# rsjahnige/CRYSTALS-Kyber

Measured on NVIDIA B200. Metric: ML-KEM-768 Encaps+Decaps ops/s, higher is better.
Workload: dtype u16/u64 integer

## Files before the change

### crystals-kyber_b200/csrc/mlkem_b200.cu

```cuda
#include "mlkem_kernels.cuh"

#include "../../include/mlkem_b200.h"

#include <algorithm>
#include <atomic>
#include <cstdio>
#include <cstdlib>
#include <cstring>
#include <mutex>
#include <vector>

namespace {

using namespace mlkem;

thread_local char tl_error[512] = "";
std::atomic<unsigned long long> g_launches{0};
int env_int(const char *name, int dflt) {
    const char *v = getenv(name);
    return v && *v ? atoi(v) : dflt;
}
constexpr int kSlots = 6;
constexpr int kDevSlots = 4;
constexpr int kHostSlots = 3;
// ... 65 lines not shown
    for (int i = 0; i < 7; i++) o |= ((r >> i) & 1u) << (6 - i);
    return o;
}
unsigned pow17(unsigned e) {
    unsigned z = 1;
    while (e--) z = (z * 17u) % kQ;
    return z;
}
uint2 shoup_pair(unsigned w) { return make_uint2(w, (w << 16) / kQ); }
uint2 shoup_pair32(unsigned w) { return make_uint2(w, (unsigned)(((unsigned long long)w << 32) / kQ)); }

void build_tables(TwiddleTables &t, uint2 rc[24]) {
    for (unsigned i = 0; i < 128; i++) {
        t.zeta[i] = shoup_pair(pow17(bitrev7(i)));
        t.gamma[i] = shoup_pair(pow17(2 * bitrev7(i) + 1));
        t.gamma32[i] = shoup_pair32(t.gamma[i].x);
        t.zeta32[i] = shoup_pair32(t.zeta[i].x);
    }
    t.zeta_inv_last[0] = shoup_pair((t.zeta[1].x * 3303u) % kQ);
    t.zeta_inv_last[1] = shoup_pair(3303u);
    t.zeta_inv_last32[0] = shoup_pair32(t.zeta_inv_last[0].x);
    t.zeta_inv_last32[1] = shoup_pair32(3303u);
    uint8_t lfsr = 1;
    for (int round = 0; round < 24; round++) {
        unsigned long long c = 0;
        for (int j = 0; j <= 6; j++) {
            if (lfsr & 1) c |= 1ULL << ((1u << j) - 1);
            uint8_t hi = lfsr & 0x80;
            lfsr = (uint8_t)(lfsr << 1);
            if (hi) lfsr ^= 0x71;
        }
        rc[round] = make_uint2((unsigned)c, (unsigned)(c >> 32));
    }
}

struct DeviceCtx {
    bool ready = false;
    cudaStream_t stream[kSlots] = {};
    void *ws[kSlots] = {};
    size_t ws_bytes[kSlots] = {};
    void *io[kSlots] = {};
    size_t io_bytes[kSlots] = {};
    cudaEvent_t ev_fork = nullptr, ev_join[kSlots] = {}, ev_slot[kSlots] = {};
    void *misc = nullptr;
    size_t misc_bytes = 0;
    int host_group = 0;
    std::mutex call_mutex;
    std::mutex misc_mutex;
};
DeviceCtx g_ctx[kMaxDevices];
std::mutex g_mutex;

struct DeviceGuard {
    int prev = -1;
    bool changed = false;
    int enter(int d) {
        if (cudaGetDevice(&prev) != cudaSuccess) prev = -1;
        if (prev == d) return 0;
        CU(cudaSetDevice(d));
        changed = true;
        return 0;
    }
    ~DeviceGuard() {
        if (changed && prev >= 0) cudaSetDevice(prev);
    }
};

// ... 19 lines not shown
    return 0;
}
template <class P>
int allow_smem_matvec() {
    const size_t b = matvec_smem_bytes<P>();
    if (int rc = allow_smem(k_sample_matvec<P, kModeKeyGen>, b)) return rc;
    if (int rc = allow_smem(k_sample_matvec<P, kModeEncrypt>, b)) return rc;
    if (int rc = allow_smem(k_sample_matvec<P, kModeEncryptCompare>, b)) return rc;
    if (int rc = allow_smem(k_sample_matvec_list<P, kModeKeyGen>, b)) return rc;
    if (int rc = allow_smem(k_sample_matvec_list<P, kModeEncrypt>, b)) return rc;
    if (int rc = allow_smem(k_sample_matvec_list<P, kModeEncryptCompare>, b)) return rc;
    return 0;
}

int acquire(const mlkem_b200_opts *o, int *dev, DeviceCtx **ctx, DeviceGuard &guard) {
    int d = o ? o->device : -1;
    if (d < 0) CU(cudaGetDevice(&d));
    if (d >= kMaxDevices) {
        snprintf(tl_error, sizeof tl_error, "device ordinal %d out of range", d);
        return MLKEM_B200_ERR_ARG;
    }
    if (int rc = guard.enter(d)) return rc;
    std::lock_guard<std::mutex> lock(g_mutex);
    DeviceCtx &c = g_ctx[d];
    if (!c.ready) {
        cudaStream_t st[kSlots] = {};
        cudaEvent_t ev[2 * kSlots + 1] = {};
        auto create = [&]() -> int {
            TwiddleTables t;
            uint2 rc[24];
            build_tables(t, rc);
            CU(cudaMemcpyToSymbol(c_tw, &t, sizeof t));
            CU(cudaMemcpyToSymbol(g_tw, &t, sizeof t));
            CU(cudaMemcpyToSymbol(c_keccak_rc, rc, sizeof rc));
            uint32_t pow2[32];
            for (int k = 0; k < 32; k++) pow2[k] = 1u << k;
            CU(cudaMemcpyToSymbol(c_pow2, pow2, sizeof pow2));
            for (int s = 0; s < kSlots; s++) CU(cudaStreamCreateWithFlags(&st[s], cudaStreamNonBlocking));
            for (int e = 0; e < 2 * kSlots + 1; e++) CU(cudaEventCreateWithFlags(&ev[e], cudaEventDisableTiming));
            if (int r = allow_smem_matvec<P512>()) return r;
            if (int r = allow_smem_matvec<P768>()) return r;
            if (int r = allow_smem_matvec<P1024>()) return r;
            if (int r = allow_smem(k_sample_ntt_batch, 128 * kSlotWords * 4)) return r;
            return 0;
        };
        if (int r = create()) {
            for (auto s_ : st)
                if (s_) cudaStreamDestroy(s_);
            for (auto e_ : ev)
                if (e_) cudaEventDestroy(e_);
            return r;
        }
        for (int s = 0; s < kSlots; s++) {
            c.stream[s] = st[s];
            c.ev_join[s] = ev[s];
            c.ev_slot[s] = ev[kSlots + s];
        }
        c.ev_fork = ev[2 * kSlots];
        c.ready = true;
    }
    *dev = d;
    *ctx = &c;
    return 0;
}

struct Arena {
    uint8_t *base;
    size_t off = 0;
    explicit Arena(void *p) : base(static_cast<uint8_t *>(p)) {}
    template <class T>
// ... 1454 lines not shown
```

### crystals-kyber_b200/csrc/mlkem_device.cuh

```cuda
#pragma once
#include <cuda_runtime.h>
#include <stdint.h>

namespace mlkem {

constexpr int kN = 256;
constexpr uint32_t kQ = 3329;
constexpr uint32_t kFullMask = 0xFFFFFFFFu;

struct TwiddleTables {
    uint2 zeta[128];
    uint2 zeta_inv_last[2];
    uint2 gamma[128];
    uint2 gamma32[128];
    uint2 zeta32[128];
    uint2 zeta_inv_last32[2];
};
__constant__ TwiddleTables c_tw;
__device__ TwiddleTables g_tw;
__constant__ uint2 c_keccak_rc[24];
__constant__ uint32_t c_pow2[32];
__device__ __forceinline__ uint32_t shl_fma(uint32_t x, int k) { return x * c_pow2[k]; }
__device__ __forceinline__ uint2 lane_zeta(int i) { return __ldg(&g_tw.zeta[i]); }
__device__ __forceinline__ uint2 lane_zeta32(int i) { return __ldg(&g_tw.zeta32[i]); }
__device__ __forceinline__ uint2 lane_gamma(int i) { return __ldg(&g_tw.gamma32[i]); }


__device__ __forceinline__ uint32_t mulhi(uint32_t a, uint32_t b) {
#ifndef MLKEM_B200_MULHI_WIDE
    return __umulhi(a, b);
#else
    [[maybe_unused]] uint32_t lo;
    uint32_t hi;
    asm volatile("{.reg .b64 t; mul.wide.u32 t, %2, %3; mov.b64 {%0, %1}, t;}" : "=r"(lo), "=r"(hi) : "r"(a), "r"(b));
    return hi;
#endif
}

__device__ __forceinline__ uint32_t mul_shoup(uint32_t a, uint2 w) {
    uint32_t qh = (a * w.y) >> 16;
    return a * w.x - qh * kQ;
}
__device__ __forceinline__ uint32_t mul_shoup_fma(uint32_t a, uint32_t w, uint32_t w32) {
    uint32_t qh = mulhi(a, w32);
    return a * w - qh * kQ;
}
constexpr bool kFmaPipe = true, kBalanced = false;
template <bool FMA>
__device__ __forceinline__ uint32_t mulz(uint32_t a, uint2 z) {
    return FMA ? mul_shoup_fma(a, z.x, z.y) : mul_shoup(a, z);
}
__device__ __forceinline__ uint32_t canon_fma(uint32_t x) { return x - mulhi(x, 1290168u) * kQ; }
__device__ __forceinline__ uint32_t barrett16(uint32_t x) {
    uint32_t qh = (x * 40317u) >> 27;
    return x - qh * kQ;
// ... 251 lines not shown
    for (int i = 0; i < 2; i++) t.z2[i] = lane_z<FMA>(127 - (2 * lane + i));
}

__device__ __forceinline__ void store_scratch_A(const uint32_t x[8], uint16_t *s, int lane) {
#pragma unroll
    for (int r = 0; r < 8; r++) s[sidx(idxA(lane, r))] = (uint16_t)x[r];
}
__device__ __forceinline__ void load_scratch_A(uint32_t x[8], const uint16_t *s, int lane) {
#pragma unroll
    for (int r = 0; r < 8; r++) x[r] = s[sidx(idxA(lane, r))];
}
__device__ __forceinline__ void store_scratch_B(const uint32_t x[8], uint16_t *s, int lane) {
#pragma unroll
    for (int r = 0; r < 8; r++) s[sidx(idxB(lane, r))] = (uint16_t)x[r];
}
__device__ __forceinline__ void load_scratch_B(uint32_t x[8], const uint16_t *s, int lane) {
#pragma unroll
    for (int r = 0; r < 8; r++) x[r] = s[sidx(idxB(lane, r))];
}
__device__ __forceinline__ uint4 pack_pairs(const uint32_t x[8]) {
    return make_uint4(x[0] + x[1] * 65536u, x[2] + x[3] * 65536u, x[4] + x[5] * 65536u, x[6] + x[7] * 65536u);
}
__device__ __forceinline__ void unpack_pairs(uint4 v, uint32_t x[8]) {
    x[0] = v.x & 0xFFFFu; x[1] = v.x >> 16; x[2] = v.y & 0xFFFFu; x[3] = v.y >> 16;
    x[4] = v.z & 0xFFFFu; x[5] = v.z >> 16; x[6] = v.w & 0xFFFFu; x[7] = v.w >> 16;
}
__device__ __forceinline__ void store_scratch_C(const uint32_t x[8], uint16_t *s, int lane) {
    *reinterpret_cast<uint4 *>(s + sidx(8 * lane)) = pack_pairs(x);
}
__device__ __forceinline__ void load_scratch_C(uint32_t x[8], const uint16_t *s, int lane) {
    unpack_pairs(*reinterpret_cast<const uint4 *>(s + sidx(8 * lane)), x);
}

template <bool FMA = false>
__device__ __forceinline__ void ct_bfly(uint32_t &a, uint32_t &b, uint2 z) {
    uint32_t t = mulz<FMA>(b, z);
    b = a - t + 2 * kQ;
    a = a + t;
}

template <bool FMA = false>
__device__ __forceinline__ void ntt_warp(uint32_t x[8], uint16_t *scratch, int lane, const LaneTwiddles &tw) {
#pragma unroll
    for (int r = 0; r < 4; r++) ct_bfly<FMA>(x[r], x[r + 4], uniform_z<FMA>(1));
#pragma unroll
    for (int h = 0; h < 2; h++)
#pragma unroll
        for (int r = 0; r < 2; r++) ct_bfly<FMA>(x[4 * h + r], x[4 * h + r + 2], uniform_z<FMA>(2 + h));
#pragma unroll
    for (int h = 0; h < 4; h++) ct_bfly<FMA>(x[2 * h], x[2 * h + 1], uniform_z<FMA>(4 + h));
    store_scratch_A(x, scratch, lane);
    __syncwarp();
    load_scratch_B(x, scratch, lane);
    __syncwarp();
#pragma unroll
    for (int r = 0; r < 4; r++) ct_bfly<FMA>(x[r], x[r + 4], tw.z16);
#pragma unroll
    for (int h = 0; h < 2; h++)
#pragma unroll
        for (int r = 0; r < 2; r++) ct_bfly<FMA>(x[4 * h + r], x[4 * h + r + 2], tw.z8[h]);
#pragma unroll
    for (int h = 0; h < 4; h++) ct_bfly<FMA>(x[2 * h], x[2 * h + 1], tw.z4[h]);
    store_scratch_B(x, scratch, lane);
    __syncwarp();
    load_scratch_C(x, scratch, lane);
    __syncwarp();
// ... 67 lines not shown
    }
#pragma unroll
    for (int h = 0; h < 2; h++)
#pragma unroll
        for (int r = 0; r < 2; r++) gs_bfly<FMA>(x[4 * h + r], x[4 * h + r + 2], tw.z8[h], 2 * kQ);
#pragma unroll
    for (int r = 0; r < 4; r++) gs_bfly<FMA>(x[r], x[r + 4], tw.z16, 4 * kQ);
    store_scratch_B(x, scratch, lane);
    __syncwarp();
    load_scratch_A(x, scratch, lane);
    __syncwarp();
#pragma unroll
    for (int h = 0; h < 4; h++) {
        gs_bfly<FMA>(x[2 * h], x[2 * h + 1], uniform_z<FMA>(7 - h), 8 * kQ);
        x[2 * h] = FMA ? barrett32(x[2 * h]) : barrett16(x[2 * h]);
    }
#pragma unroll
    for (int h = 0; h < 2; h++)
#pragma unroll
        for (int r = 0; r < 2; r++) gs_bfly<FMA>(x[4 * h + r], x[4 * h + r + 2], uniform_z<FMA>(3 - h), 2 * kQ);
    const uint2 zs = FMA ? c_tw.zeta_inv_last32[1] : c_tw.zeta_inv_last[1], zl = FMA ? c_tw.zeta_inv_last32[0] : c_tw.zeta_inv_last[0];
#pragma unroll
    for (int r = 0; r < 4; r++) {
        uint32_t t = x[r];
        x[r] = mulz<FMA>(t + x[r + 4], zs);
        x[r + 4] = mulz<FMA>(x[r + 4] - t + 4 * kQ, zl);
        if (CANON) {
            x[r] = csubq(x[r]);
            x[r + 4] = csubq(x[r + 4]);
        }
    }
}

__device__ __forceinline__ void basemul_acc(uint32_t &acc0, uint32_t &acc1, uint32_t a0, uint32_t a1, uint32_t b0,
                                            uint32_t b1, uint2 gamma) {
    uint32_t a1g = mul_shoup_fma(a1, gamma.x, gamma.y);
    acc0 += a0 * b0 + a1g * b1;
    acc1 += a0 * b1 + a1 * b0;
}

template <int D>
__device__ __forceinline__ void pack8(const uint32_t v[8], uint8_t *dst) {
    constexpr int NW = (8 * D + 31) / 32;
    uint32_t w[NW];
#pragma unroll
    for (int k = 0; k < NW; k++) {
        uint32_t acc = 0;
#pragma unroll
        for (int i = 0; i < 8; i++) {
            const int off = D * i - 32 * k;
            if (off >= 0 && off < 32) acc += v[i] * (1u << off);
            else if (off < 0 && off + D > 0) acc += v[i] >> (-off);
        }
        w[k] = acc;
    }
    if (D % 4 == 0) {
#pragma unroll
        for (int k = 0; k < NW; k++) reinterpret_cast<uint32_t *>(dst)[k] = w[k];
    } else if (D % 2 == 0) {
#pragma unroll
        for (int h = 0; h < D / 2; h++) reinterpret_cast<uint16_t *>(dst)[h] = (uint16_t)(w[h >> 1] >> (16 * (h & 1)));
    } else {
#pragma unroll
        for (int b8 = 0; b8 < D; b8++) dst[b8] = (uint8_t)(w[b8 >> 2] >> (8 * (b8 & 3)));
    }
}
// ... 51 lines not shown
```

### crystals-kyber_b200/csrc/mlkem_kernels.cuh

```cuda
#pragma once
#include "mlkem_device.cuh"

namespace mlkem {

template <int K_, int ETA1_, int ETA2_, int DU_, int DV_>
struct ParamSet {
    static constexpr int K = K_, ETA1 = ETA1_, ETA2 = ETA2_, DU = DU_, DV = DV_;
    static constexpr int EK = 384 * K + 32;
    static constexpr int DKPKE = 384 * K;
    static constexpr int DK = 768 * K + 96;
    static constexpr int C1ROW = 32 * DU;
    static constexpr int C2 = 32 * DV;
    static constexpr int C = C1ROW * K + C2;
};
using P512 = ParamSet<2, 3, 2, 10, 4>;
using P768 = ParamSet<3, 2, 2, 10, 4>;
using P1024 = ParamSet<4, 2, 2, 11, 5>;

struct KeySel {
    const uint32_t *index;
    uint32_t base, nkeys;
};
__device__ __forceinline__ size_t key_row(const KeySel &k, int item) {
    if (k.index) return min(__ldg(k.index + item), k.nkeys - 1u);
// ... 373 lines not shown
        keccak_f1600(a);
        int next = 0;
        if (LEFT) {
            cbd3_words(carry, a[0].lo, a[0].hi, o0, o1);
            put(2 * G1, o0);
            put(2 * G1 + 1, o1);
            next = 2;
        }
#pragma unroll
        for (int g = G1 + (LEFT ? 1 : 0); g < 16; g++) {
            const int w = next + 3 * (g - G1 - (LEFT ? 1 : 0));
            uint32_t w0 = (w & 1) ? a[w >> 1].hi : a[w >> 1].lo, w1 = ((w + 1) & 1) ? a[(w + 1) >> 1].hi : a[(w + 1) >> 1].lo,
                     w2 = ((w + 2) & 1) ? a[(w + 2) >> 1].hi : a[(w + 2) >> 1].lo;
            cbd3_words(w0, w1, w2, o0, o1);
            put(2 * g, o0);
            put(2 * g + 1, o1);
        }
    }
}

__device__ __forceinline__ void store_layoutC_global(const uint32_t x[8], int lane, uint16_t *dst) {
    reinterpret_cast<uint4 *>(dst)[lane] = pack_pairs(x);
}
__device__ __forceinline__ void load_layoutC_global(uint32_t x[8], int lane, const uint16_t *src) {
    unpack_pairs(__ldg(reinterpret_cast<const uint4 *>(src) + lane), x);
}

template <int ETA, bool NTT_OUT, int RATE = kRateShake128>
__global__ void __launch_bounds__(kNoiseTPB) k_noise(int n, const uint8_t *__restrict__ seeds, size_t seed_stride, int nonce0,
                                                     uint16_t *__restrict__ out16, size_t out16_stride,
                                                     uint32_t *__restrict__ outc, size_t outc_stride,
                                                     uint8_t *__restrict__ enc12, size_t enc12_stride, int enc12_polys) {
    __shared__ uint32_t s_codes[NTT_OUT ? kNoiseTPB * 33 : 1];
    __shared__ __align__(16) uint16_t s_scratch[NTT_OUT ? (kNoiseTPB / 32) * kScratchU16 : 2];
    const int p = blockIdx.y;
    const int item = blockIdx.x * kNoiseTPB + threadIdx.x;
    Lane seed[4];
#pragma unroll
    for (int w = 0; w < 4; w++) seed[w] = item < n ? load_lane(seeds + seed_stride * item + 8 * w) : Lane{0u, 0u};
    if (NTT_OUT) {
        uint32_t *mine = s_codes + 33 * threadIdx.x;
        prf_cbd_codes<ETA, RATE>(seed, (uint32_t)(nonce0 + p), [&](int w, uint32_t v) { mine[w] = v; });
        __syncwarp();
        const int lane = threadIdx.x & 31, warp = threadIdx.x >> 5;
        uint16_t *scratch = s_scratch + warp * kScratchU16;
        LaneTwiddles tw;
        load_lane_twiddles<kFmaPipe>(tw, lane);
        const uint32_t pw = nibble_weight(lane & 7);
        for (int t = 0; t < 32; t++) {
            int it = blockIdx.x * kNoiseTPB + warp * 32 + t;
            if (it >= n) break;
            const uint32_t *codes = s_codes + 33 * (warp * 32 + t) + (lane >> 3);
            uint32_t x[8];
#pragma unroll
            for (int r = 0; r < 8; r++) x[r] = nibble_fma(codes[4 * r], pw) + (kQ - 3);
            ntt_warp<kFmaPipe>(x, scratch, lane, tw);
            store_layoutC_global(x, lane, out16 + out16_stride * it + 256 * p);
            if (p < enc12_polys) {
                uint32_t *row = reinterpret_cast<uint32_t *>(enc12 + enc12_stride * it + 384 * p) + 3 * lane;
                row[0] = x[0] | (x[1] << 12) | (x[2] << 24);
                row[1] = (x[2] >> 8) | (x[3] << 4) | (x[4] << 16) | (x[5] << 28);
                row[2] = (x[5] >> 4) | (x[6] << 8) | (x[7] << 20);
            }
        }
    } else {
        if (item >= n) return;
        uint32_t buf[32];
        prf_cbd_codes<ETA, RATE>(seed, (uint32_t)(nonce0 + p), [&](int w, uint32_t v) { buf[w] = v; });
        uint4 *dst = reinterpret_cast<uint4 *>(outc + outc_stride * item + 32 * p);
#pragma unroll
        for (int v = 0; v < 8; v++) dst[v] = make_uint4(buf[4 * v], buf[4 * v + 1], buf[4 * v + 2], buf[4 * v + 3]);
    }
}

template <bool CHECKED>
__device__ __forceinline__ void parse_block(const Lane a[25], uint32_t &addr, uint32_t end_addr) {
#pragma unroll
    for (int ch = 0; ch < 7; ch++) {
        const uint32_t w[7] = {a[3 * ch].lo, a[3 * ch].hi, a[3 * ch + 1].lo, a[3 * ch + 1].hi, a[3 * ch + 2].lo, a[3 * ch + 2].hi, 0u};
#pragma unroll
        for (int m = 0; m < 16; m++) {
            const int bit = 12 * m, wi = bit >> 5, sh = bit & 31;
            uint32_t t;
            if (sh == 20) t = w[wi];
            else if (sh < 20) t = w[wi] * (1u << (20 - sh));
            else t = __funnelshift_r(w[wi], w[wi + 1], sh - 20);
            bool ok = t < (kQ << 20);
            if (CHECKED) ok = ok && (addr < end_addr);
            uint32_t d;
            asm("mul.hi.u32 %0, %1, 4096;" : "=r"(d) : "r"(t));
            if (ok) {
                asm volatile("st.shared.u16 [%0], %1;" ::"r"(addr), "h"((uint16_t)d) : "memory");
                addr += 2;
            }
        }
    }
// ... 991 lines not shown
```

Before: 33.71 million.

## Compute noise-polynomial NTT with int8 tensor-core MMA instead of butterflies

The noise kernel's NTT_OUT path replaces the per-warp butterfly NTT with a dense 128x128 matrix product on int8 tensor cores (mma m16n8k32 u8.s8). The CBD nibble codes feed the A operand directly and the NTT matrix is split into signed low and high byte limbs, with a precomputed bias absorbing the -3 offset and keeping the result positive. This removes shared-memory scratch shuffles and butterfly arithmetic in exchange for far more MACs per polynomial and loads of B fragments from global memory. A standalone microbenchmark comparing MMA and butterfly NTT is also added.

```diff
diff --git a/crystals-kyber_b200/csrc/mlkem_b200.cu b/crystals-kyber_b200/csrc/mlkem_b200.cu
--- a/crystals-kyber_b200/csrc/mlkem_b200.cu
+++ b/crystals-kyber_b200/csrc/mlkem_b200.cu
@@ -121,6 +121,37 @@
         }
         rc[round] = make_uint2((unsigned)c, (unsigned)(c >> 32));
     }
+}
+
+void build_mma_frags(uint2 *frag, bool inverse, uint32_t *noise_bias) {
+    static int m[128][128];
+    for (unsigned i = 0; i < 128; i++)
+        for (unsigned j = 0; j < 128; j++) {
+            const unsigned e = ((2 * bitrev7(i) + 1) * j) % 256;
+            int v = inverse ? (int)(3303u * pow17(255 * e % 256) % kQ) : (int)pow17(e);
+            if (v > (int)kQ / 2) v -= kQ;
+            if (inverse) m[j][i] = v;
+            else m[i][j] = v;
+        }
+    for (int nt = 0; nt < 16; nt++)
+        for (int kt = 0; kt < 4; kt++)
+            for (int limb = 0; limb < 2; limb++)
+                for (int lane = 0; lane < 32; lane++) {
+                    unsigned w[2] = {0, 0};
+                    for (int reg = 0; reg < 2; reg++)
+                        for (int e = 0; e < 4; e++) {
+                            const int c = m[8 * nt + (lane >> 2)][32 * kt + 16 * reg + 4 * (lane & 3) + e];
+                            const int lo = ((c + 128) & 255) - 128, hi = (c - lo) >> 8;
+                            w[reg] |= (unsigned)((limb ? hi : lo) & 255) << (8 * e);
+                        }
+                    frag[((nt * 4 + kt) * 2 + limb) * 32 + lane] = make_uint2(w[0], w[1]);
+                }
+    if (noise_bias)
+        for (int i = 0; i < 128; i++) {
+            int s = 0;
+            for (int j = 0; j < 128; j++) s += m[i][j];
+            noise_bias[i] = (unsigned)((int)kQ * 256 - 3 * s);
+        }
 }
 
 struct DeviceCtx {
@@ -207,6 +238,9 @@
             build_tables(t, rc);
             CU(cudaMemcpyToSymbol(c_tw, &t, sizeof t));
             CU(cudaMemcpyToSymbol(g_tw, &t, sizeof t));
+            static MmaNttTables mt;
+            build_mma_frags(mt.ntt_frag, false, mt.noise_bias);
+            CU(cudaMemcpyToSymbol(g_mma, &mt, sizeof mt));
             CU(cudaMemcpyToSymbol(c_keccak_rc, rc, sizeof rc));
             uint32_t pow2[32];
             for (int k = 0; k < 32; k++) pow2[k] = 1u << k;
diff --git a/crystals-kyber_b200/csrc/mlkem_device.cuh b/crystals-kyber_b200/csrc/mlkem_device.cuh
--- a/crystals-kyber_b200/csrc/mlkem_device.cuh
+++ b/crystals-kyber_b200/csrc/mlkem_device.cuh
@@ -21,6 +21,12 @@
 __constant__ uint2 c_keccak_rc[24];
 __constant__ uint32_t c_pow2[32];
 __device__ __forceinline__ uint32_t shl_fma(uint32_t x, int k) { return x * c_pow2[k]; }
+constexpr int kNttFragWords = 16 * 4 * 2 * 32;
+struct MmaNttTables {
+    uint2 ntt_frag[kNttFragWords];
+    uint32_t noise_bias[128];
+};
+__device__ MmaNttTables g_mma;
 __device__ __forceinline__ uint2 lane_zeta(int i) { return __ldg(&g_tw.zeta[i]); }
 __device__ __forceinline__ uint2 lane_zeta32(int i) { return __ldg(&g_tw.zeta32[i]); }
 __device__ __forceinline__ uint2 lane_gamma(int i) { return __ldg(&g_tw.gamma32[i]); }
@@ -338,6 +344,12 @@
     unpack_pairs(*reinterpret_cast<const uint4 *>(s + sidx(8 * lane)), x);
 }
 
+__device__ __forceinline__ void mma_u8s8(int (&d)[4], const uint32_t (&a)[4], uint2 b) {
+    asm volatile("mma.sync.aligned.m16n8k32.row.col.s32.u8.s8.s32 {%0,%1,%2,%3}, {%4,%5,%6,%7}, {%8,%9}, {%0,%1,%2,%3};"
+                 : "+r"(d[0]), "+r"(d[1]), "+r"(d[2]), "+r"(d[3])
+                 : "r"(a[0]), "r"(a[1]), "r"(a[2]), "r"(a[3]), "r"(b.x), "r"(b.y));
+}
+
 template <bool FMA = false>
 __device__ __forceinline__ void ct_bfly(uint32_t &a, uint32_t &b, uint2 z) {
     uint32_t t = mulz<FMA>(b, z);
diff --git a/crystals-kyber_b200/csrc/mlkem_kernels.cuh b/crystals-kyber_b200/csrc/mlkem_kernels.cuh
--- a/crystals-kyber_b200/csrc/mlkem_kernels.cuh
+++ b/crystals-kyber_b200/csrc/mlkem_kernels.cuh
@@ -429,7 +429,6 @@
                                                      uint32_t *__restrict__ outc, size_t outc_stride,
                                                      uint8_t *__restrict__ enc12, size_t enc12_stride, int enc12_polys) {
     __shared__ uint32_t s_codes[NTT_OUT ? kNoiseTPB * 33 : 1];
-    __shared__ __align__(16) uint16_t s_scratch[NTT_OUT ? (kNoiseTPB / 32) * kScratchU16 : 2];
     const int p = blockIdx.y;
     const int item = blockIdx.x * kNoiseTPB + threadIdx.x;
     Lane seed[4];
@@ -439,26 +438,65 @@
         uint32_t *mine = s_codes + 33 * threadIdx.x;
         prf_cbd_codes<ETA, RATE>(seed, (uint32_t)(nonce0 + p), [&](int w, uint32_t v) { mine[w] = v; });
         __syncwarp();
-        const int lane = threadIdx.x & 31, warp = threadIdx.x >> 5;
-        uint16_t *scratch = s_scratch + warp * kScratchU16;
-        LaneTwiddles tw;
-        load_lane_twiddles<kFmaPipe>(tw, lane);
-        const uint32_t pw = nibble_weight(lane & 7);
-        for (int t = 0; t < 32; t++) {
-            int it = blockIdx.x * kNoiseTPB + warp * 32 + t;
-            if (it >= n) break;
-            const uint32_t *codes = s_codes + 33 * (warp * 32 + t) + (lane >> 3);
-            uint32_t x[8];
-#pragma unroll
-            for (int r = 0; r < 8; r++) x[r] = nibble_fma(codes[4 * r], pw) + (kQ - 3);
-            ntt_warp<kFmaPipe>(x, scratch, lane, tw);
-            store_layoutC_global(x, lane, out16 + out16_stride * it + 256 * p);
-            if (p < enc12_polys) {
-                uint32_t *row = reinterpret_cast<uint32_t *>(enc12 + enc12_stride * it + 384 * p) + 3 * lane;
-                row[0] = x[0] | (x[1] << 12) | (x[2] << 24);
-                row[1] = (x[2] >> 8) | (x[3] << 4) | (x[4] << 16) | (x[5] << 28);
-                row[2] = (x[5] >> 4) | (x[6] << 8) | (x[7] << 20);
+        const int lane = threadIdx.x & 31, warp = threadIdx.x >> 5, g = lane >> 2, t = lane & 3;
+        uint32_t a[2][4][2][4];
+#pragma unroll
+        for (int mt = 0; mt < 2; mt++)
+#pragma unroll
+            for (int kt = 0; kt < 4; kt++)
+#pragma unroll
+                for (int reg = 0; reg < 4; reg++) {
+                    const uint32_t w = s_codes[33 * (warp * 32 + 16 * mt + g + 8 * (reg & 1)) + 8 * kt + 4 * (reg >> 1) + t];
+                    a[mt][kt][0][reg] = w & 0x0F0F0F0Fu;
+                    a[mt][kt][1][reg] = (w >> 4) & 0x0F0F0F0Fu;
+                }
+        const int it0 = blockIdx.x * kNoiseTPB + warp * 32;
+#pragma unroll 1
+        for (int nt = 0; nt < 16; nt++) {
+            const uint2 bias = __ldg(reinterpret_cast<const uint2 *>(g_mma.noise_bias + 8 * nt + 2 * t));
+            int acc[2][2][2][4];
+#pragma unroll
+            for (int mt = 0; mt < 2; mt++)
+#pragma unroll
+                for (int b = 0; b < 2; b++) {
+                    acc[mt][b][0][0] = acc[mt][b][0][2] = (int)bias.x;
+                    acc[mt][b][0][1] = acc[mt][b][0][3] = (int)bias.y;
+                    acc[mt][b][1][0] = acc[mt][b][1][1] = acc[mt][b][1][2] = acc[mt][b][1][3] = 0;
+                }
+#pragma unroll
+            for (int kt = 0; kt < 4; kt++) {
+                const uint2 bl = __ldg(&g_mma.ntt_frag[((nt * 4 + kt) * 2 + 0) * 32 + lane]);
+                const uint2 bh = __ldg(&g_mma.ntt_frag[((nt * 4 + kt) * 2 + 1) * 32 + lane]);
+#pragma unroll
+                for (int mt = 0; mt < 2; mt++)
+#pragma unroll
+                    for (int b = 0; b < 2; b++) {
+                        mma_u8s8(acc[mt][b][0], a[mt][kt][b], bl);
+                        mma_u8s8(acc[mt][b][1], a[mt][kt][b], bh);
+                    }
             }
+#pragma unroll
+            for (int mt = 0; mt < 2; mt++)
+#pragma unroll
+                for (int half = 0; half < 2; half++) {
+                    const int it = it0 + 16 * mt + g + 8 * half;
+                    uint32_t y[4];
+#pragma unroll
+                    for (int c = 0; c < 2; c++)
+#pragma unroll
+                        for (int b = 0; b < 2; b++)
+                            y[2 * c + b] = canon_fma((uint32_t)acc[mt][b][0][2 * half + c] + (uint32_t)acc[mt][b][1][2 * half + c] * 256u);
+                    if (it < n) {
+                        *reinterpret_cast<uint2 *>(out16 + out16_stride * it + 256 * p + 16 * nt + 4 * t) =
+                            make_uint2(y[0] + y[1] * 65536u, y[2] + y[3] * 65536u);
+                        if (p < enc12_polys) {
+                            uint16_t *row = reinterpret_cast<uint16_t *>(enc12 + enc12_stride * it + 384 * p + 24 * nt + 6 * t);
+                            row[0] = (uint16_t)(y[0] | (y[1] << 12));
+                            row[1] = (uint16_t)((y[1] >> 4) | (y[2] << 8));
+                            row[2] = (uint16_t)((y[2] >> 8) | (y[3] << 4));
+                        }
+                    }
+                }
         }
     } else {
         if (item >= n) return;
diff --git a/crystals-kyber_b200/csrc/mma_ntt_bench.cu b/crystals-kyber_b200/csrc/mma_ntt_bench.cu
--- /dev/null
+++ b/crystals-kyber_b200/csrc/mma_ntt_bench.cu
@@ -0,0 +1,241 @@
+#include "mlkem_b200.cu"
+
+#include <vector>
+
+using namespace mlkem;
+
+#define CK(x)                                                                                        \
+    do {                                                                                             \
+        cudaError_t e_ = (x);                                                                        \
+        if (e_ != cudaSuccess) {                                                                     \
+            fprintf(stderr, "CUDA error %s at %s:%d\n", cudaGetErrorString(e_), __FILE__, __LINE__); \
+            exit(2);                                                                                 \
+        }                                                                                            \
+    } while (0)
+
+__device__ __forceinline__ void imma(int (&d)[4], const uint32_t (&a)[4], uint32_t b0, uint32_t b1) {
+    mma_u8s8(d, a, make_uint2(b0, b1));
+}
+
+template <int CHAINS>
+__global__ void __launch_bounds__(256) k_imma_rate(int iters, int *out, unsigned long long *cycles) {
+    int d[CHAINS][4];
+    uint32_t a[4] = {threadIdx.x, threadIdx.x * 3u, threadIdx.x ^ 0x55u, blockIdx.x};
+    uint32_t b0 = threadIdx.x * 7u, b1 = blockIdx.x * 5u;
+#pragma unroll
+    for (int c = 0; c < CHAINS; c++) d[c][0] = d[c][1] = d[c][2] = d[c][3] = c;
+    unsigned long long t0 = clock64();
+    for (int i = 0; i < iters; i++) {
+#pragma unroll
+        for (int c = 0; c < CHAINS; c++) imma(d[c], a, b0, b1);
+    }
+    unsigned long long t1 = clock64();
+    int acc = 0;
+#pragma unroll
+    for (int c = 0; c < CHAINS; c++) acc ^= d[c][0] ^ d[c][1] ^ d[c][2] ^ d[c][3];
+    if (acc == 0x12345678) out[0] = acc;
+    if (threadIdx.x == 0) cycles[blockIdx.x] = t1 - t0;
+}
+
+template <int CHAINS>
+static void run_imma(const char *name, int sms, int blocks_per_sm, int threads, int *d_out, unsigned long long *d_cyc) {
+    const int iters = 8192, blocks = sms * blocks_per_sm;
+    cudaEvent_t e0, e1;
+    CK(cudaEventCreate(&e0));
+    CK(cudaEventCreate(&e1));
+    k_imma_rate<CHAINS><<<blocks, threads>>>(64, d_out, d_cyc);
+    CK(cudaDeviceSynchronize());
+    float best = 1e30f;
+    double cyc = 0;
+    for (int rep = 0; rep < 3; rep++) {
+        CK(cudaEventRecord(e0));
+        k_imma_rate<CHAINS><<<blocks, threads>>>(iters, d_out, d_cyc);
+        CK(cudaEventRecord(e1));
+        CK(cudaEventSynchronize(e1));
+        float ms;
+        CK(cudaEventElapsedTime(&ms, e0, e1));
+        if (ms < best) {
+            best = ms;
+            std::vector<unsigned long long> h(blocks);
+            CK(cudaMemcpy(h.data(), d_cyc, blocks * sizeof(unsigned long long), cudaMemcpyDeviceToHost));
+            cyc = 0;
+            for (auto c : h) cyc += (double)c;
+            cyc /= blocks;
+        }
+    }
+    const double warps_per_sm = blocks_per_sm * threads / 32.0;
+    const double mma_per_sm = warps_per_sm * (double)iters * CHAINS;
+    const double total_mac = (double)blocks * threads / 32.0 * iters * CHAINS * 4096.0;
+    printf("  \"%s\": {\"warps_per_sm\": %.0f, \"chains_per_warp\": %d, \"imma_per_clk_per_sm\": %.4f, "
+           "\"clk_per_imma_per_warp\": %.2f, \"int8_tera_mac_per_s\": %.1f, \"ms\": %.4f},\n",
+           name, warps_per_sm, CHAINS, mma_per_sm / cyc, cyc / ((double)iters * CHAINS), total_mac / (best * 1e-3) / 1e12,
+           best);
+    CK(cudaEventDestroy(e0));
+    CK(cudaEventDestroy(e1));
+}
+
+constexpr int kMmaTPB = 256;
+constexpr int kFragWords = 2 * kNttFragWords;
+
+__device__ __forceinline__ void split_limbs(uint4 v, uint32_t &el, uint32_t &eh, uint32_t &ol, uint32_t &oh) {
+    const uint32_t lo01 = __byte_perm(v.x, v.y, 0x6420), lo23 = __byte_perm(v.z, v.w, 0x6420);
+    const uint32_t hi01 = __byte_perm(v.x, v.y, 0x7531), hi23 = __byte_perm(v.z, v.w, 0x7531);
+    el = __byte_perm(lo01, lo23, 0x6420);
+    eh = __byte_perm(hi01, hi23, 0x6420);
+    ol = __byte_perm(lo01, lo23, 0x7531);
+    oh = __byte_perm(hi01, hi23, 0x7531);
+}
+
+__global__ void __launch_bounds__(kMmaTPB) k_ntt_mma(int n, const uint16_t *__restrict__ in, uint16_t *__restrict__ out,
+                                                     const uint2 *__restrict__ frags, int mask12) {
+    __shared__ uint2 s_frag[kFragWords / 2];
+    for (int i = threadIdx.x; i < kFragWords / 2; i += kMmaTPB) s_frag[i] = frags[i];
+    __syncthreads();
+    const int lane = threadIdx.x & 31, warp = threadIdx.x >> 5, g = lane >> 2, t = lane & 3;
+    const int tiles = n / 16;
+    for (int tile = blockIdx.x * (kMmaTPB / 32) + warp; tile < tiles; tile += gridDim.x * (kMmaTPB / 32)) {
+        const uint16_t *src = in + (size_t)256 * 16 * tile;
+        uint32_t a[4][2][2][4];
+#pragma unroll
+        for (int kt = 0; kt < 4; kt++) {
+#pragma unroll
+            for (int reg = 0; reg < 4; reg++) {
+                const int row = g + 8 * (reg & 1), half = reg >> 1;
+                uint4 v = __ldg(reinterpret_cast<const uint4 *>(src + 256 * row + 64 * kt + 32 * half + 8 * t));
+                if (mask12) {
+                    v.x &= 0x0FFF0FFFu; v.y &= 0x0FFF0FFFu; v.z &= 0x0FFF0FFFu; v.w &= 0x0FFF0FFFu;
+                }
+                split_limbs(v, a[kt][0][0][reg], a[kt][0][1][reg], a[kt][1][0][reg], a[kt][1][1][reg]);
+            }
+        }
+        uint16_t *dst = out + (size_t)256 * 16 * tile;
+#pragma unroll 1
+        for (int nt = 0; nt < 16; nt++) {
+            int acc[2][3][4];
+#pragma unroll
+            for (int p = 0; p < 2; p++)
+#pragma unroll
+                for (int w = 0; w < 3; w++)
+#pragma unroll
+                    for (int r = 0; r < 4; r++) acc[p][w][r] = w == 0 ? (int)(kQ << 18) : 0;
+#pragma unroll
+            for (int kt = 0; kt < 4; kt++) {
+                const uint2 bl = s_frag[((nt * 4 + kt) * 2 + 0) * 32 + lane], bh = s_frag[((nt * 4 + kt) * 2 + 1) * 32 + lane];
+#pragma unroll
+                for (int p = 0; p < 2; p++) {
+                    imma(acc[p][0], a[kt][p][0], bl.x, bl.y);
+                    imma(acc[p][1], a[kt][p][0], bh.x, bh.y);
+                    imma(acc[p][1], a[kt][p][1], bl.x, bl.y);
+                    imma(acc[p][2], a[kt][p][1], bh.x, bh.y);
+                }
+            }
+            uint32_t y[2][4];
+#pragma unroll
+            for (int p = 0; p < 2; p++)
+#pragma unroll
+                for (int r = 0; r < 4; r++)
+                    y[p][r] = canon32((uint32_t)acc[p][0][r] + (uint32_t)acc[p][1][r] * 256u + (uint32_t)acc[p][2][r] * 65536u);
+            *reinterpret_cast<uint2 *>(dst + 256 * g + 16 * nt + 4 * t) = make_uint2(y[0][0] | y[1][0] << 16, y[0][1] | y[1][1] << 16);
+            *reinterpret_cast<uint2 *>(dst + 256 * (g + 8) + 16 * nt + 4 * t) =
+                make_uint2(y[0][2] | y[1][2] << 16, y[0][3] | y[1][3] << 16);
+        }
+    }
+}
+
+static std::vector<uint2> make_frags(bool inverse) {
+    std::vector<uint2> f(kFragWords / 2);
+    build_mma_frags(f.data(), inverse, nullptr);
+    return f;
+}
+
+template <class Launch>
+static float time_ms(Launch launch, int reps) {
+    cudaEvent_t e0, e1;
+    CK(cudaEventCreate(&e0));
+    CK(cudaEventCreate(&e1));
+    CK(cudaEventRecord(e0));
+    for (int r = 0; r < reps; r++) launch();
+    CK(cudaEventRecord(e1));
+    CK(cudaEventSynchronize(e1));
+    float ms;
+    CK(cudaEventElapsedTime(&ms, e0, e1));
+    CK(cudaEventDestroy(e0));
+    CK(cudaEventDestroy(e1));
+    return ms / reps;
+}
+
+int main() {
+    cudaDeviceProp prop;
+    CK(cudaGetDeviceProperties(&prop, 0));
+    const int sms = prop.multiProcessorCount;
+    int clk_khz = 0;
+    CK(cudaDeviceGetAttribute(&clk_khz, cudaDevAttrClockRate, 0));
+    printf("{\n  \"gpu\": \"%s\", \"sms\": %d, \"max_sm_khz\": %d,\n", prop.name, sms, clk_khz);
+
+    int *d_out;
+    unsigned long long *d_cyc;
+    CK(cudaMalloc(&d_out, 64));
+    CK(cudaMalloc(&d_cyc, sizeof(unsigned long long) * sms * 8));
+    run_imma<1>("imma_latency_1warp_per_smsp", sms, 1, 128, d_out, d_cyc);
+    run_imma<8>("imma_1warp_per_smsp_8chains", sms, 1, 128, d_out, d_cyc);
+    run_imma<4>("imma_4warps_per_smsp_4chains", sms, 2, 256, d_out, d_cyc);
+    run_imma<8>("imma_8warps_per_smsp_8chains", sms, 4, 256, d_out, d_cyc);
+
+    TwiddleTables tw;
+    uint2 rc[24];
+    build_tables(tw, rc);
+    CK(cudaMemcpyToSymbol(c_tw, &tw, sizeof tw));
+    CK(cudaMemcpyToSymbol(g_tw, &tw, sizeof tw));
+
+    const int n = 1 << 20;
+    std::vector<uint16_t> h(256 * (size_t)n);
+    uint64_t s = 0x9E3779B97F4A7C15ull;
+    for (auto &v : h) {
+        s ^= s << 13; s ^= s >> 7; s ^= s << 17;
+        v = (uint16_t)(s % kQ);
+    }
+    uint16_t *d_in, *d_ref, *d_mma;
+    uint2 *d_fwd, *d_inv;
+    CK(cudaMalloc(&d_in, 512ull * n));
+    CK(cudaMalloc(&d_ref, 512ull * n));
+    CK(cudaMalloc(&d_mma, 512ull * n));
+    CK(cudaMemcpy(d_in, h.data(), 512ull * n, cudaMemcpyHostToDevice));
+    auto fwd = make_frags(false), inv = make_frags(true);
+    CK(cudaMalloc(&d_fwd, fwd.size() * sizeof(uint2)));
+    CK(cudaMalloc(&d_inv, inv.size() * sizeof(uint2)));
+    CK(cudaMemcpy(d_fwd, fwd.data(), fwd.size() * sizeof(uint2), cudaMemcpyHostToDevice));
+    CK(cudaMemcpy(d_inv, inv.data(), inv.size() * sizeof(uint2), cudaMemcpyHostToDevice));
+
+    int occ_bfly = 0, occ_mma = 0;
+    CK(cudaOccupancyMaxActiveBlocksPerMultiprocessor(&occ_bfly, k_ntt_batch, kPrimTPB, 0));
+    CK(cudaOccupancyMaxActiveBlocksPerMultiprocessor(&occ_mma, k_ntt_mma, kMmaTPB, 0));
+    const int grid_bfly = sms * occ_bfly, grid_mma = sms * occ_mma;
+    std::vector<uint16_t> a(256 * (size_t)n), b(256 * (size_t)n);
+    for (int inverse = 0; inverse < 2; inverse++) {
+        auto bfly = [&]() {
+            if (inverse) k_intt_batch<<<grid_bfly, kPrimTPB>>>(n, d_in, d_ref);
+            else k_ntt_batch<<<grid_bfly, kPrimTPB>>>(n, d_in, d_ref);
+        };
+        auto mma = [&]() { k_ntt_mma<<<grid_mma, kMmaTPB>>>(n, d_in, d_mma, inverse ? d_inv : d_fwd, inverse); };
+        bfly();
+        mma();
+        CK(cudaDeviceSynchronize());
+        CK(cudaMemcpy(a.data(), d_ref, 512ull * n, cudaMemcpyDeviceToHost));
+        CK(cudaMemcpy(b.data(), d_mma, 512ull * n, cudaMemcpyDeviceToHost));
+        size_t bad = 0;
+        for (size_t i = 0; i < a.size(); i++) bad += a[i] != b[i];
+        float tb[5], tm[5];
+        for (int r = 0; r < 5; r++) {
+            tb[r] = time_ms(bfly, 10);
+            tm[r] = time_ms(mma, 10);
+        }
+        auto mn = [](float *x) { float m = x[0]; for (int i = 1; i < 5; i++) m = std::min(m, x[i]); return m; };
+        auto mx = [](float *x) { float m = x[0]; for (int i = 1; i < 5; i++) m = std::max(m, x[i]); return m; };
+        printf("  \"%s\": {\"polys\": %d, \"mismatches\": %zu, \"butterfly_ms\": [%.4f, %.4f], \"mma_ms\": [%.4f, %.4f], "
+               "\"butterfly_G_polys_per_s\": %.3f, \"mma_G_polys_per_s\": %.3f, \"blocks_per_sm\": [%d, %d]}%s\n",
+               inverse ? "intt" : "ntt", n, bad, mn(tb), mx(tb), mn(tm), mx(tm), n / (mn(tb) * 1e6), n / (mn(tm) * 1e6),
+               occ_bfly, occ_mma, inverse ? "" : ",");
+    }
+    printf("}\n");
+    return 0;
+}
```

New measurement: 34.40 million, median of 6. +2.0%, better.

## Compute noise-polynomial forward NTT as int8 tensor-core matrix multiply

Applied to the files above, without the earlier changes.

Adds a tensor-core path that computes the forward NTT of CBD noise polynomials as a dense matrix product. It uses mma.sync m16n8k32 s8 with a precomputed twiddle matrix split into low and high 6-bit signed limbs, plus a per-row correction constant. The path is enabled by default for noise polys that are not also byte-encoded, and processes 8 items per warp per pass. It replaces the shuffle/shared-memory butterfly NTT with far more MACs on otherwise idle tensor cores, at the cost of global table loads and extra reductions. A standalone tensor-core throughput microbenchmark is also added.

```diff
diff --git a/crystals-kyber_b200/csrc/mlkem_b200.cu b/crystals-kyber_b200/csrc/mlkem_b200.cu
--- a/crystals-kyber_b200/csrc/mlkem_b200.cu
+++ b/crystals-kyber_b200/csrc/mlkem_b200.cu
@@ -122,6 +122,34 @@
         rc[round] = make_uint2((unsigned)c, (unsigned)(c >> 32));
     }
 }
+
+#if MLKEM_B200_TC_TRANSFORMS
+void build_tc_ntt_table(TcNttTable &tb) {
+    auto centered = [](unsigned i, unsigned j) {
+        const int v = (int)pow17(((2 * bitrev7(i) + 1) * j) % 256);
+        return v > (int)kQ / 2 ? v - (int)kQ : v;
+    };
+    for (unsigned i = 0; i < 128; i++) {
+        long s = 0;
+        for (unsigned j = 0; j < 128; j++) s += centered(i, j);
+        tb.kcorr[i] = (unsigned)(((-3 * s) % (long)kQ + kQ) % kQ) + 394u * kQ;
+    }
+    for (int m = 0; m < 8; m++)
+        for (int kk = 0; kk < 4; kk++)
+            for (int lane = 0; lane < 32; lane++) {
+                const int g = lane >> 2, t = lane & 3;
+                unsigned w[2][4] = {};
+                for (int r = 0; r < 4; r++)
+                    for (int b = 0; b < 4; b++) {
+                        const int v = centered(16 * m + g + 8 * (r & 1), 32 * kk + 4 * t + 16 * (r >> 1) + b);
+                        const int lo = ((v + 32) & 63) - 32, hi = (v - lo) / 64;
+                        w[0][r] |= (unsigned)(lo & 0xFF) << (8 * b);
+                        w[1][r] |= (unsigned)(hi & 0xFF) << (8 * b);
+                    }
+                for (int l = 0; l < 2; l++) tb.frag[m][kk][l][lane] = make_uint4(w[l][0], w[l][1], w[l][2], w[l][3]);
+            }
+}
+#endif
 
 struct DeviceCtx {
     bool ready = false;
@@ -211,6 +239,11 @@
             uint32_t pow2[32];
             for (int k = 0; k < 32; k++) pow2[k] = 1u << k;
             CU(cudaMemcpyToSymbol(c_pow2, pow2, sizeof pow2));
+#if MLKEM_B200_TC_TRANSFORMS
+            static TcNttTable tc;
+            build_tc_ntt_table(tc);
+            CU(cudaMemcpyToSymbol(g_tc_ntt, &tc, sizeof tc));
+#endif
             for (int s = 0; s < kSlots; s++) CU(cudaStreamCreateWithFlags(&st[s], cudaStreamNonBlocking));
             for (int e = 0; e < 2 * kSlots + 1; e++) CU(cudaEventCreateWithFlags(&ev[e], cudaEventDisableTiming));
             if (int r = allow_smem_matvec<P512>()) return r;
diff --git a/crystals-kyber_b200/csrc/mlkem_device.cuh b/crystals-kyber_b200/csrc/mlkem_device.cuh
--- a/crystals-kyber_b200/csrc/mlkem_device.cuh
+++ b/crystals-kyber_b200/csrc/mlkem_device.cuh
@@ -471,6 +471,53 @@
     }
 }
 
+#ifndef MLKEM_B200_TC_TRANSFORMS
+#define MLKEM_B200_TC_TRANSFORMS 1
+#endif
+struct TcNttTable {
+    uint4 frag[8][4][2][32];
+    uint32_t kcorr[128];
+};
+__device__ TcNttTable g_tc_ntt;
+
+__device__ __forceinline__ void mma_s8_16832(int (&c)[4], uint4 a, uint32_t b0, uint32_t b1) {
+    asm volatile("mma.sync.aligned.m16n8k32.row.col.s32.s8.s8.s32 {%0,%1,%2,%3}, {%4,%5,%6,%7}, {%8,%9}, {%0,%1,%2,%3};"
+                 : "+r"(c[0]), "+r"(c[1]), "+r"(c[2]), "+r"(c[3])
+                 : "r"(a.x), "r"(a.y), "r"(a.z), "r"(a.w), "r"(b0), "r"(b1));
+}
+template <typename CODES, typename PUT>
+__device__ __forceinline__ void ntt_tc_codes8(int lane, CODES codes, PUT put) {
+    const int g = lane >> 2, t = lane & 3;
+    uint32_t be[4][2], bo[4][2];
+#pragma unroll
+    for (int kk = 0; kk < 4; kk++)
+#pragma unroll
+        for (int h = 0; h < 2; h++) {
+            const uint32_t w = codes(g, 8 * kk + 4 * h + t);
+            be[kk][h] = w & 0x0F0F0F0Fu;
+            bo[kk][h] = (w >> 4) & 0x0F0F0F0Fu;
+        }
+#pragma unroll 1
+    for (int m = 0; m < 8; m++) {
+        const uint32_t k0 = __ldg(&g_tc_ntt.kcorr[16 * m + g]), k1 = __ldg(&g_tc_ntt.kcorr[16 * m + g + 8]);
+        int el[4] = {(int)k0, (int)k0, (int)k1, (int)k1}, ol[4] = {(int)k0, (int)k0, (int)k1, (int)k1};
+        int eh[4] = {0, 0, 0, 0}, oh[4] = {0, 0, 0, 0};
+#pragma unroll
+        for (int kk = 0; kk < 4; kk++) {
+            const uint4 al = __ldg(&g_tc_ntt.frag[m][kk][0][lane]), ah = __ldg(&g_tc_ntt.frag[m][kk][1][lane]);
+            mma_s8_16832(el, al, be[kk][0], be[kk][1]);
+            mma_s8_16832(eh, ah, be[kk][0], be[kk][1]);
+            mma_s8_16832(ol, al, bo[kk][0], bo[kk][1]);
+            mma_s8_16832(oh, ah, bo[kk][0], bo[kk][1]);
+        }
+#pragma unroll
+        for (int e = 0; e < 4; e++) {
+            const uint32_t ve = csubq(barrett32((uint32_t)(el[e] + 64 * eh[e]))), vo = csubq(barrett32((uint32_t)(ol[e] + 64 * oh[e])));
+            put(2 * t + (e & 1), 16 * m + g + 8 * (e >> 1), ve + vo * 65536u);
+        }
+    }
+}
+
 __device__ __forceinline__ void basemul_acc(uint32_t &acc0, uint32_t &acc1, uint32_t a0, uint32_t a1, uint32_t b0,
                                             uint32_t b1, uint2 gamma) {
     uint32_t a1g = mul_shoup_fma(a1, gamma.x, gamma.y);
diff --git a/crystals-kyber_b200/csrc/mlkem_kernels.cuh b/crystals-kyber_b200/csrc/mlkem_kernels.cuh
--- a/crystals-kyber_b200/csrc/mlkem_kernels.cuh
+++ b/crystals-kyber_b200/csrc/mlkem_kernels.cuh
@@ -440,6 +440,21 @@
         prf_cbd_codes<ETA, RATE>(seed, (uint32_t)(nonce0 + p), [&](int w, uint32_t v) { mine[w] = v; });
         __syncwarp();
         const int lane = threadIdx.x & 31, warp = threadIdx.x >> 5;
+#if MLKEM_B200_TC_TRANSFORMS
+        if (p >= enc12_polys) {
+            for (int t0 = 0; t0 < 32; t0 += 8) {
+                const int it0 = blockIdx.x * kNoiseTPB + warp * 32 + t0;
+                if (it0 >= n) break;
+                const uint32_t *base = s_codes + 33 * (warp * 32 + t0);
+                ntt_tc_codes8(
+                    lane, [&](int q8, int w) { return base[33 * q8 + w]; },
+                    [&](int q8, int i, uint32_t v) {
+                        if (it0 + q8 < n) reinterpret_cast<uint32_t *>(out16 + out16_stride * (it0 + q8) + 256 * p)[i] = v;
+                    });
+            }
+            return;
+        }
+#endif
         uint16_t *scratch = s_scratch + warp * kScratchU16;
         LaneTwiddles tw;
         load_lane_twiddles<kFmaPipe>(tw, lane);
diff --git a/crystals-kyber_b200/csrc/tc_bench.cu b/crystals-kyber_b200/csrc/tc_bench.cu
--- /dev/null
+++ b/crystals-kyber_b200/csrc/tc_bench.cu
@@ -0,0 +1,282 @@
+#include <cuda_runtime.h>
+
+#include <cstdint>
+#include <cstdio>
+#include <cstdlib>
+#include <cstring>
+#include <string>
+#include <vector>
+
+#define CK(x)                                                                                        \
+    do {                                                                                             \
+        cudaError_t e_ = (x);                                                                        \
+        if (e_ != cudaSuccess) {                                                                     \
+            fprintf(stderr, "CUDA error %s at %s:%d\n", cudaGetErrorString(e_), __FILE__, __LINE__); \
+            exit(2);                                                                                 \
+        }                                                                                            \
+    } while (0)
+
+enum T { T_NONE = 0, T_MMA_REG, T_MMA_LDSM, T_TC05_N64, T_TC05_N128, T_TC05_N256, T_HMMA_REG, T_HMMA_LDSM, T_COUNT };
+static const char *kName[T_COUNT] = {"none", "mma.sync m16n8k32 s8, A in registers", "mma.sync m16n8k32 s8, A by ldmatrix.x4 per MMA",
+                                     "tcgen05.mma kind::i8 M128 K128 N64", "tcgen05.mma kind::i8 M128 K128 N128",
+                                     "tcgen05.mma kind::i8 M128 K128 N256", "mma.sync m16n8k16 f16 -> f32, A in registers",
+                                     "mma.sync m16n8k16 f16 -> f32, A by ldmatrix.x4 per MMA"};
+static constexpr int kTcN[T_COUNT] = {0, 0, 0, 64, 128, 256, 0, 0};
+
+constexpr int kFragBytes = 512;
+constexpr int kFrags = 64;
+constexpr int kSmemA = 4096 * 4;
+constexpr int kSmemB = 256 * 128;
+constexpr int kOffOperands = 1024;
+constexpr size_t kDynSmem = 200 * 1024;
+
+__device__ __forceinline__ uint32_t smem_u32(const void *p) { return (uint32_t)__cvta_generic_to_shared(p); }
+
+__device__ __forceinline__ void mma_s8(int (&c)[4], const uint32_t (&a)[4], uint32_t b0, uint32_t b1) {
+    asm volatile("mma.sync.aligned.m16n8k32.row.col.s32.s8.s8.s32 {%0,%1,%2,%3}, {%4,%5,%6,%7}, {%8,%9}, {%0,%1,%2,%3};"
+                 : "+r"(c[0]), "+r"(c[1]), "+r"(c[2]), "+r"(c[3])
+                 : "r"(a[0]), "r"(a[1]), "r"(a[2]), "r"(a[3]), "r"(b0), "r"(b1));
+}
+__device__ __forceinline__ void mma_f16(float (&c)[4], const uint32_t (&a)[4], uint32_t b0, uint32_t b1) {
+    asm volatile("mma.sync.aligned.m16n8k16.row.col.f32.f16.f16.f32 {%0,%1,%2,%3}, {%4,%5,%6,%7}, {%8,%9}, {%0,%1,%2,%3};"
+                 : "+f"(c[0]), "+f"(c[1]), "+f"(c[2]), "+f"(c[3])
+                 : "r"(a[0]), "r"(a[1]), "r"(a[2]), "r"(a[3]), "r"(b0), "r"(b1));
+}
+__device__ __forceinline__ void ldsm_x4(uint32_t (&a)[4], uint32_t addr) {
+    asm volatile("ldmatrix.sync.aligned.m8n8.x4.shared.b16 {%0,%1,%2,%3}, [%4];" : "=r"(a[0]), "=r"(a[1]), "=r"(a[2]), "=r"(a[3]) : "r"(addr) : "memory");
+}
+
+__device__ __forceinline__ uint64_t sdesc(uint32_t addr, uint32_t lbo, uint32_t sbo) {
+    return (uint64_t)((addr >> 4) & 0x3FFFu) | ((uint64_t)((lbo >> 4) & 0x3FFFu) << 16) | ((uint64_t)((sbo >> 4) & 0x3FFFu) << 32) | (1ull << 46);
+}
+__host__ __device__ constexpr uint32_t idesc_i8(int m, int n) {
+    return (2u << 4) | (1u << 7) | (1u << 10) | ((uint32_t)(n >> 3) << 17) | ((uint32_t)(m >> 4) << 24);
+}
+__device__ __forceinline__ void tc05_mma(uint32_t tmem, uint64_t a, uint64_t b, uint32_t idesc, uint32_t acc) {
+    asm volatile("{.reg .pred p; setp.ne.u32 p, %4, 0; tcgen05.mma.cta_group::1.kind::i8 [%0], %1, %2, %3, p;}" ::"r"(tmem), "l"(a), "l"(b), "r"(idesc), "r"(acc));
+}
+
+template <int TOP>
+__global__ void __launch_bounds__(256, 1) k(uint32_t *out, int lop3_iters, int t_iters, unsigned long long *res) {
+    extern __shared__ __align__(1024) uint8_t smem[];
+    volatile int *done = reinterpret_cast<volatile int *>(smem);
+    uint32_t *tmem_slot = reinterpret_cast<uint32_t *>(smem + 16);
+    uint64_t *bar = reinterpret_cast<uint64_t *>(smem + 32);
+    uint8_t *ops = smem + kOffOperands;
+    const int warp = threadIdx.x >> 5, lane = threadIdx.x & 31;
+    const bool is_a = warp < 4;
+    constexpr bool kTc05 = TOP >= T_TC05_N64 && TOP <= T_TC05_N256;
+    constexpr int kN = kTcN[TOP];
+    for (int i = threadIdx.x; i < (kSmemA + kSmemB) / 4; i += blockDim.x) reinterpret_cast<uint32_t *>(ops)[i] = out[4] * i;
+    if (threadIdx.x == 0) {
+        *done = 0;
+        asm volatile("mbarrier.init.shared::cta.b64 [%0], 1;" ::"r"(smem_u32(bar)));
+        asm volatile("fence.mbarrier_init.release.cluster;" ::: "memory");
+    }
+    if (kTc05 && warp == 4) {
+        asm volatile("tcgen05.alloc.cta_group::1.sync.aligned.shared::cta.b32 [%0], %1;" ::"r"(smem_u32(tmem_slot)), "r"(kN) : "memory");
+        asm volatile("tcgen05.relinquish_alloc_permit.cta_group::1.sync.aligned;");
+    }
+    asm volatile("fence.proxy.async.shared::cta;" ::: "memory");
+    __syncthreads();
+    asm volatile("tcgen05.fence::after_thread_sync;" ::: "memory");
+    const bool lop3 = lop3_iters > 0;
+    unsigned long long t0 = clock64(), count = 0;
+    uint32_t x0 = threadIdx.x, x1 = x0 + 1, x2 = x0 + 2, x3 = x0 + 3, x4 = x0 + 4, x5 = x0 + 5, x6 = x0 + 6, x7 = x0 + 7;
+    const uint32_t m = out[0] | 0x10001u, s = (out[1] & 7) + 3;
+    if (is_a) {
+        if (lop3) {
+            for (int i = 0; i < lop3_iters; i++) {
+#pragma unroll
+                for (int r = 0; r < 4; r++) {
+#define L3(a) asm volatile("lop3.b32 %0, %0, %1, %2, 0x96;" : "+r"(a) : "r"(m), "r"(s));
+                    L3(x0) L3(x1) L3(x2) L3(x3) L3(x4) L3(x5) L3(x6) L3(x7)
+#undef L3
+                }
+            }
+            count = (unsigned long long)lop3_iters * 32;
+            __syncwarp();
+            if (lane == 0) atomicAdd((int *)done, 1);
+        }
+    } else if (TOP == T_MMA_REG || TOP == T_MMA_LDSM) {
+        int c[8][4];
+#pragma unroll
+        for (int a = 0; a < 8; a++) c[a][0] = c[a][1] = c[a][2] = c[a][3] = 0;
+        uint32_t fa[4] = {out[4], out[4] + 1, out[4] + 2, out[4] + 3}, b0 = out[4], b1 = out[4] + 7;
+        const uint32_t abase = smem_u32(ops) + (lane >> 3) * 128 + (lane & 7) * 16;
+        int f = 0, it = 0;
+        while (lop3 ? *done < 4 : it < t_iters) {
+#pragma unroll
+            for (int a = 0; a < 8; a++) {
+                if (TOP == T_MMA_LDSM) ldsm_x4(fa, abase + ((f + a) & (kFrags - 1)) * kFragBytes);
+                mma_s8(c[a], fa, b0, b1);
+            }
+            f = (f + 8) & (kFrags - 1);
+            it++;
+            count += 8;
+        }
+        int acc = 0;
+#pragma unroll
+        for (int a = 0; a < 8; a++) acc ^= c[a][0] ^ c[a][1] ^ c[a][2] ^ c[a][3];
+        if (acc == 0x12345678) out[3] = acc;
+    } else if (TOP == T_HMMA_REG || TOP == T_HMMA_LDSM) {
+        float c[8][4];
+#pragma unroll
+        for (int a = 0; a < 8; a++) c[a][0] = c[a][1] = c[a][2] = c[a][3] = 0.f;
+        uint32_t fa[4] = {out[4], out[4], out[4], out[4]}, b0 = out[4], b1 = out[4];
+        const uint32_t abase = smem_u32(ops) + (lane >> 3) * 128 + (lane & 7) * 16;
+        int f = 0, it = 0;
+        while (lop3 ? *done < 4 : it < t_iters) {
+#pragma unroll
+            for (int a = 0; a < 8; a++) {
+                if (TOP == T_HMMA_LDSM) ldsm_x4(fa, abase + ((f + a) & (kFrags - 1)) * kFragBytes);
+                mma_f16(c[a], fa, b0, b1);
+            }
+            f = (f + 8) & (kFrags - 1);
+            it++;
+            count += 8;
+        }
+        float acc = 0.f;
+#pragma unroll
+        for (int a = 0; a < 8; a++) acc += c[a][0] + c[a][1] + c[a][2] + c[a][3];
+        if (acc == 1234.5f) out[3] = 1;
+    } else if (kTc05 && warp == 4) {
+        const uint32_t tmem = *tmem_slot, abase = smem_u32(ops), bbase = abase + kSmemA;
+        constexpr uint32_t kLbo = 128, kSbo = 1024;
+        constexpr uint32_t idesc = idesc_i8(128, kN);
+        if (lane == 0) {
+            int it = 0;
+            while (lop3 ? *done < 4 : it < t_iters) {
+#pragma unroll
+                for (int kk = 0; kk < 4; kk++)
+                    tc05_mma(tmem, sdesc(abase + kk * 256, kLbo, kSbo), sdesc(bbase + kk * 256, kLbo, kSbo), idesc, (it | kk) != 0);
+                it++;
+                count += 4;
+            }
+            asm volatile("tcgen05.commit.cta_group::1.mbarrier::arrive::one.shared::cluster.b64 [%0];" ::"r"(smem_u32(bar)) : "memory");
+            asm volatile(
+                "{.reg .pred p; W: mbarrier.try_wait.parity.shared::cta.b64 p, [%0], 0; @!p bra W;}" ::"r"(smem_u32(bar))
+                : "memory");
+        }
+        __syncwarp();
+        count = __shfl_sync(0xFFFFFFFFu, count, 0);
+    }
+    unsigned long long t1 = clock64();
+    asm volatile("tcgen05.fence::before_thread_sync;" ::: "memory");
+    uint32_t accx = x0 ^ x1 ^ x2 ^ x3 ^ x4 ^ x5 ^ x6 ^ x7;
+    if (accx == 0x12345678u) out[3] = accx;
+    if (lane == 0) {
+        res[(blockIdx.x * 8 + warp) * 2] = t1 - t0;
+        res[(blockIdx.x * 8 + warp) * 2 + 1] = count;
+    }
+    __syncthreads();
+    if (kTc05 && warp == 4) {
+        asm volatile("tcgen05.fence::after_thread_sync;" ::: "memory");
+        asm volatile("tcgen05.dealloc.cta_group::1.sync.aligned.b32 %0, %1;" ::"r"(*tmem_slot), "r"(kN) : "memory");
+    }
+}
+
+static std::string g_card = "unknown", g_power = "unknown", g_clock = "unknown";
+
+static void query_card() {
+    FILE *p = popen("nvidia-smi --query-gpu=name,power.limit,clocks.sm,clocks.max.sm --format=csv,noheader -i 0 2>/dev/null", "r");
+    if (!p) return;
+    char line[512] = {0};
+    if (fgets(line, sizeof line, p)) {
+        std::vector<std::string> f;
+        std::string cur;
+        for (char *c = line; *c && *c != '\n'; c++) {
+            if (*c == ',') {
+                f.push_back(cur);
+                cur.clear();
+            } else if (!(cur.empty() && *c == ' ')) {
+                cur += *c;
+            }
+        }
+        f.push_back(cur);
+        if (f.size() >= 4) {
+            g_card = f[0];
+            g_power = f[1];
+            g_clock = f[2] + " (max " + f[3] + ")";
+        }
+    }
+    pclose(p);
+}
+
+template <int TOP>
+static void run(int sms, bool with_lop3, uint32_t *d_out, unsigned long long *d_res) {
+    const int lop3_iters = with_lop3 ? 20000 : 0;
+    const bool tc05 = TOP >= T_TC05_N64 && TOP <= T_TC05_N256;
+    const int t_iters = tc05 ? 2000 * 256 / kTcN[TOP] : 20000;
+    CK(cudaFuncSetAttribute(k<TOP>, cudaFuncAttributeMaxDynamicSharedMemorySize, (int)kDynSmem));
+    k<TOP><<<sms, 256, kDynSmem>>>(d_out, with_lop3 ? 100 : 0, 20, d_res);
+    CK(cudaDeviceSynchronize());
+    cudaEvent_t e0, e1;
+    CK(cudaEventCreate(&e0));
+    CK(cudaEventCreate(&e1));
+    CK(cudaEventRecord(e0));
+    k<TOP><<<sms, 256, kDynSmem>>>(d_out, lop3_iters, t_iters, d_res);
+    CK(cudaEventRecord(e1));
+    CK(cudaDeviceSynchronize());
+    float ms = 0;
+    CK(cudaEventElapsedTime(&ms, e0, e1));
+    std::vector<unsigned long long> h((size_t)sms * 16);
+    CK(cudaMemcpy(h.data(), d_res, h.size() * sizeof(unsigned long long), cudaMemcpyDeviceToHost));
+    const double mac_per_instr = tc05 ? 128.0 * kTcN[TOP] * 32 : (TOP >= T_HMMA_REG) ? 16.0 * 8 * 16 : 16.0 * 8 * 32;
+    double lop3_ipc = 0, t_instr = 0, t_macs_per_clk = 0;
+    for (int b = 0; b < sms; b++) {
+        double tcyc = 0, tcnt = 0;
+        for (int w = 0; w < 8; w++) {
+            const double cyc = (double)h[(b * 8 + w) * 2], cnt = (double)h[(b * 8 + w) * 2 + 1];
+            if (w < 4) {
+                if (with_lop3) lop3_ipc += cnt / cyc;
+            } else {
+                tcyc = cyc > tcyc ? cyc : tcyc;
+                tcnt += cnt;
+            }
+        }
+        t_instr += tcnt;
+        if (tcyc > 0) t_macs_per_clk += tcnt * mac_per_instr / tcyc;
+    }
+    lop3_ipc /= sms * 4;
+    t_macs_per_clk /= sms;
+    const double t_tops = t_instr * mac_per_instr * 2 / (ms * 1e-3) / 1e12;
+    printf("{\"card\": \"%s\", \"power_limit\": \"%s\", \"sm_clock\": \"%s\", \"tensor_stream\": \"%s\", \"with_lop3_warps\": %s, "
+           "\"tensor_macs_per_clk_per_sm\": %.1f, \"tensor_T_op_per_s\": %.1f, \"lop3_warp_ipc\": %.4f, \"kernel_ms\": %.3f}\n",
+           g_card.c_str(), g_power.c_str(), g_clock.c_str(), kName[TOP], with_lop3 ? "true" : "false", t_macs_per_clk,
+           TOP == T_NONE ? 0.0 : t_tops, lop3_ipc, ms);
+    fflush(stdout);
+    CK(cudaEventDestroy(e0));
+    CK(cudaEventDestroy(e1));
+}
+
+int main(int argc, char **argv) {
+    const bool no_tc05 = argc > 1 && strcmp(argv[1], "--no-tcgen05") == 0;
+    query_card();
+    cudaDeviceProp prop;
+    CK(cudaGetDeviceProperties(&prop, 0));
+    uint32_t *d_out;
+    unsigned long long *d_res;
+    CK(cudaMalloc(&d_out, 64));
+    CK(cudaMemset(d_out, 0, 64));
+    CK(cudaMalloc(&d_res, sizeof(unsigned long long) * prop.multiProcessorCount * 16));
+    const int sms = prop.multiProcessorCount;
+    run<T_NONE>(sms, true, d_out, d_res);
+    run<T_MMA_REG>(sms, false, d_out, d_res);
+    run<T_MMA_REG>(sms, true, d_out, d_res);
+    run<T_MMA_LDSM>(sms, false, d_out, d_res);
+    run<T_MMA_LDSM>(sms, true, d_out, d_res);
+    run<T_HMMA_REG>(sms, false, d_out, d_res);
+    run<T_HMMA_REG>(sms, true, d_out, d_res);
+    run<T_HMMA_LDSM>(sms, false, d_out, d_res);
+    run<T_HMMA_LDSM>(sms, true, d_out, d_res);
+    if (!no_tc05) {
+        run<T_TC05_N64>(sms, false, d_out, d_res);
+        run<T_TC05_N128>(sms, false, d_out, d_res);
+        run<T_TC05_N256>(sms, false, d_out, d_res);
+        run<T_TC05_N64>(sms, true, d_out, d_res);
+        run<T_TC05_N128>(sms, true, d_out, d_res);
+        run<T_TC05_N256>(sms, true, d_out, d_res);
+    }
+    return 0;
+}
```

New measurement: 33.70 million before, 34.26 million after (median of 6 runs). 1.02x the previous value.
